# set-soft/ComfyUI-FLOAT_Optimized

Measured on AMD Instinct MI355X. Metric: 512x512 frames/sec end-to-end audio->video @50 ODE steps, higher is better.
Workload: dtype fp16; 1 GPU; configs[1]: 10 s audio + 512x512 portrait in HBM -> 250 frames in pinned host memory; appearance encoder + wav2vec2 audio encoder + FMT sampling (50 Euler evaluations/window, CFG a=2.0 e=1.0) + decode + D2H, through InferenceAgent.infer_device (the product call); nfe=51, frames_per_clip=250, fmt_dtype=fp16, dec_dtype=fp16, decode_batch=32, hip_graph=True, parallelism=replicas x1 (one clip per GPU), stage_overlap=off

## Files before the change

comfyui-float_optimized_amd/csrc/dec_kernels.hpp:

```cpp
#pragma once
#include "common.hpp"
#include <type_traits>

constexpr int kDecSatSites = 40;
typedef unsigned short dec_us2 __attribute__((ext_vector_type(2)));
typedef _Float16 dec_h2 __attribute__((ext_vector_type(2)));
template <class T>
__device__ __forceinline__ unsigned dec_cvt2(float a, float b, unsigned& m) {
  static_assert(T::is_fp16, "fp16 path");
  const unsigned u = __builtin_bit_cast(unsigned, dec_h2{(_Float16)a, (_Float16)b});
#ifndef DEC_NO_SAT
  m = __builtin_bit_cast(unsigned, __builtin_elementwise_max(__builtin_bit_cast(dec_us2, m), __builtin_bit_cast(dec_us2, u & 0x7fff7fffu)));
#endif
  return u;
}
template <class T>
__device__ __forceinline__ void dec_sat_flush(unsigned long long* ctr, unsigned& m) {
  if constexpr (T::is_fp16) {
    if ((m & 0xffffu) >= 0x7c00u || (m >> 16) >= 0x7c00u) atomicAdd(ctr, 1ull);
    m = 0u;
  }
}
template <class T>
__device__ __forceinline__ void dec_store4(typename T::elem* p, float a, float b, float c, float d, unsigned& m) {
// ... 1192 lines not shown
  issue(0);
  for (int chunk = 0; chunk < nchunks; ++chunk) {
    __syncthreads();
#pragma unroll
    for (int i = 0; i < NA; ++i) {
      const int e = tid + i * 256, p = e >> 2, ch = e & 3;
      if (p < NPIX) *reinterpret_cast<P8*>(sA + p * RB + (ch ^ ((p >> 1) & 3)) * CB) = ra[i];
    }
#pragma unroll
    for (int i = 0; i < NB; ++i) {
      const int e = tid + i * 256;
      if (e < NBC) {
        const int row = e >> 2, ch = e & 3;
        *reinterpret_cast<P8*>(sB + row * RB + (ch ^ ((row >> 1) & 3)) * CB) = rb[i];
      }
    }
    __syncthreads();
    if (chunk + 1 < nchunks) issue(chunk + 1);
    constexpr int kNum[4] = {1, 2, 2, 4};
    constexpr int kTap[4][4] = {{0, 0, 0, 0}, {1, 4, 0, 0}, {2, 6, 0, 0}, {3, 5, 7, 8}};
    constexpr int kCls[4][4] = {{0, 0, 0, 0}, {0, 1, 0, 0}, {0, 2, 0, 0}, {0, 1, 2, 3}};
#pragma unroll
    for (int sh = 0; sh < 4; ++sh) {
      P8 a[4];
#pragma unroll
      for (int mt = 0; mt < 4; ++mt)
        a[mt] = *reinterpret_cast<const P8*>(sA + ((sh & 1) ? (aaddr[mt][sh >> 1] >> 16) : (aaddr[mt][sh >> 1] & 0xffffu)));
#pragma unroll
      for (int u = 0; u < 4; ++u) {
        if (u < kNum[sh]) {
          const int t = kTap[sh][u], c = kCls[sh][u];
          P8 b[NT];
#pragma unroll
          for (int j = 0; j < NT; ++j) b[j] = *reinterpret_cast<const P8*>(sB + baddr + (t * BN + j * 16) * RB);
#pragma unroll
          for (int mt = 0; mt < 4; ++mt)
#pragma unroll
            for (int j = 0; j < NT; ++j) acc[c][mt][j] = T::mfma(b[j], a[mt], acc[c][mt][j]);
        }
      }
    }
  }
  float4 ed[NT];
  unsigned sm = 0u;
#pragma unroll
  for (int j = 0; j < NT; ++j) ed[j] = *reinterpret_cast<const float4*>(g.demod + (size_t)f * g.ldd + n0 + j * 16 + q * 4);
#pragma unroll
  for (int mt = 0; mt < 4; ++mt) {
    const int mpos = ty * 16 + w * 4 + mt, npos = tx * 16 + r16;
#pragma unroll
    for (int c = 0; c < 4; ++c) {
      const int u = 2 * mpos + (c >> 1), v = 2 * npos + (c & 1);
      if (u >= g.OH || v >= g.OW) continue;
      E* yp = reinterpret_cast<E*>(g.Y) + ((size_t)(f * g.OH + u) * g.OW + v) * g.Cout;
#pragma unroll
      for (int j = 0; j < NT; ++j) {
        const int co = n0 + j * 16 + q * 4;
        const float4 d = ed[j];
        dec_store4<T>(yp + co, acc[c][mt][j][0] * d.x, acc[c][mt][j][1] * d.y, acc[c][mt][j][2] * d.z, acc[c][mt][j][3] * d.w, sm);
      }
    }
  }
  dec_sat_flush<T>(g.sat, sm);
}

template <class T>
__global__ __launch_bounds__(256, T::is32 ? 1 : 2) void dec_zblur_kernel(ConvArgs g) {
  DEC_COPY_PROLOGUE(g, bid)
  DEC_PH_BEGIN
  typedef typename T::elem E;
  typedef typename T::pack8 P8;
  typedef float v2f __attribute__((ext_vector_type(2)));
  constexpr int EB = T::EB, RB = 32 * EB, CB = 8 * EB;
  constexpr int NT = 2, BN = 32, HW = 17, NPIX = HW * HW, NTAPS = 9;
  constexpr int NA = (NPIX * 4 + 255) / 256, NBROWS = NTAPS * BN, NB = (NBROWS * 4 + 255) / 256;
  extern __shared__ __attribute__((aligned(16))) unsigned char smem[];
  unsigned char* const sA = smem;
  unsigned char* const sB = smem + NPIX * RB;
  unsigned char* const sZ = smem;
  const int tid = threadIdx.x, lane = tid & 63, w = __builtin_amdgcn_readfirstlane(tid >> 6);
  const int r16 = lane & 15, q = lane >> 4;
  const int Wi = g.Wi, Cin = g.Cin;
  const int tiles_pf = g.tiles_x * g.tiles_y;
  unsigned grp = bid, cb = blockIdx.y;
  if (g.ncb) dec_group_cb(bid, g.ngroups, g.ncb, grp, cb);
  const int f = (int)grp / tiles_pf, rem = (int)grp - f * tiles_pf;
  const int ty = rem / g.tiles_x, tx = rem - ty * g.tiles_x;
  const int n0 = cb * BN;
  const int nchunks = Cin >> 5;
  const int iy0 = ty * 14 - 2, ix0 = tx * 14 - 2;

  const int ch = tid & 3;
  const bool interior = iy0 >= 0 && iy0 + HW <= g.Hi && ix0 >= 0 && ix0 + HW <= Wi;
  unsigned a_off[NA], a_lds[NA], a_bad = 0u;
#pragma unroll
  for (int i = 0; i < NA; ++i) {
    const int p = min((tid >> 2) + 64 * i, NPIX - 1);
    const int hy = p / HW, hx = p - hy * HW;
    const bool in = (unsigned)(iy0 + hy) < (unsigned)g.Hi && (unsigned)(ix0 + hx) < (unsigned)Wi;
    a_off[i] = (unsigned)((((in ? hy : 2) * Wi + (in ? hx : 2)) * Cin + ch * 8) * EB);
    a_lds[i] = (unsigned)(p * RB + (ch ^ ((hx >> 1) & 3)) * CB);
    a_bad |= (in ? 0u : 1u) << i;
  }
  const unsigned char* const Xo = reinterpret_cast<const unsigned char*>(g.X) + ((long long)(f * g.Hi + iy0) * Wi + ix0) * Cin * EB;
  const int brow = tid >> 2;
  const unsigned b_off = (unsigned)((((brow / BN) * g.Cout + brow % BN) * Cin + ch * 8) * EB);
  const int brow_l = min(brow + 64 * (NB - 1), NBROWS - 1);
  const unsigned b_off_l = (unsigned)((((brow_l / BN) * g.Cout + brow_l % BN) * Cin + ch * 8) * EB);
  const unsigned b_lds = (unsigned)(brow * RB + (ch ^ ((brow >> 1) & 3)) * CB);
  const unsigned b_lds_l = (unsigned)(brow_l * RB + (ch ^ ((brow_l >> 1) & 3)) * CB);
  const size_t b_round = (size_t)(64 / BN) * g.Cout * Cin * EB;
  const unsigned char* const Wn = reinterpret_cast<const unsigned char*>(g.Wt) + (size_t)n0 * Cin * EB;
  unsigned fa[2];
#pragma unroll
  for (int dx = 0; dx < 2; ++dx) fa[dx] = (unsigned)(((w * 4) * HW + r16 + dx) * RB + (q ^ (((r16 + dx) >> 1) & 3)) * CB);
  const unsigned fb = (unsigned)(r16 * RB + (q ^ ((r16 >> 1) & 3)) * CB);

  f32x4 acc[4][4][NT];
#pragma unroll
  for (int c = 0; c < 4; ++c)
#pragma unroll
    for (int i = 0; i < 4; ++i)
#pragma unroll
      for (int j = 0; j < NT; ++j) acc[c][i][j] = f32x4{0.f, 0.f, 0.f, 0.f};

  P8 ra[NA], rb[NB];
  float dm[NT];
  float4 b4, s4;
  auto issue = [&](int chunk) {
    const unsigned char* const Xc = Xo + (size_t)(chunk << 5) * EB;
#pragma unroll
    for (int i = 0; i < NA; ++i) ra[i] = *reinterpret_cast<const P8*>(Xc + a_off[i]);
    const unsigned char* const Wc = Wn + (size_t)(chunk << 5) * EB;
#pragma unroll
    for (int i = 0; i < NB - 1; ++i) rb[i] = *reinterpret_cast<const P8*>(Wc + i * b_round + b_off);
    rb[NB - 1] = *reinterpret_cast<const P8*>(Wc + b_off_l);
  };
  issue(0);
  DEC_PH(0);
  for (int chunk = 0; chunk < nchunks; ++chunk) {
    __syncthreads();
    if (interior) {
#pragma unroll
      for (int i = 0; i < NA; ++i) *reinterpret_cast<P8*>(sA + a_lds[i]) = ra[i];
    } else {
#pragma unroll
      for (int i = 0; i < NA; ++i) *reinterpret_cast<P8*>(sA + a_lds[i]) = ((a_bad >> i) & 1u) ? T::zero8() : ra[i];
    }
#pragma unroll
    for (int i = 0; i < NB - 1; ++i) *reinterpret_cast<P8*>(sB + b_lds + i * 64 * RB) = rb[i];
    *reinterpret_cast<P8*>(sB + b_lds_l) = rb[NB - 1];
    __syncthreads();
    DEC_PH(1);
    if (chunk + 1 < nchunks) {
      issue(chunk + 1);
    } else {
#pragma unroll
      for (int j = 0; j < NT; ++j) dm[j] = g.demod[(size_t)f * g.ldd + n0 + j * 16 + r16];
      const int co = n0 + (w & 1) * 16 + q * 4;
      b4 = *reinterpret_cast<const float4*>(g.bias + co);
      s4 = *reinterpret_cast<const float4*>(g.snext + (size_t)f * g.lds + co);
    }
    constexpr int kNum[4] = {1, 2, 2, 4};
    constexpr int kTap[4][4] = {{0, 0, 0, 0}, {1, 4, 0, 0}, {2, 6, 0, 0}, {3, 5, 7, 8}};
    constexpr int kCls[4][4] = {{0, 0, 0, 0}, {0, 1, 0, 0}, {0, 2, 0, 0}, {0, 1, 2, 3}};
#pragma unroll
    for (int sh = 0; sh < 4; ++sh) {
      P8 a[4];
#pragma unroll
      for (int mt = 0; mt < 4; ++mt) a[mt] = *reinterpret_cast<const P8*>(sA + fa[sh & 1] + (mt + (sh >> 1)) * HW * RB);
#pragma unroll
      for (int u = 0; u < 4; ++u) {
        if (u < kNum[sh]) {
          const int t = kTap[sh][u], c = kCls[sh][u];
          P8 b[NT];
#pragma unroll
          for (int j = 0; j < NT; ++j) b[j] = *reinterpret_cast<const P8*>(sB + fb + (t * BN + j * 16) * RB);
#pragma unroll
          for (int mt = 0; mt < 4; ++mt)
#pragma unroll
            for (int j = 0; j < NT; ++j) acc[c][mt][j] = T::mfma(a[mt], b[j], acc[c][mt][j]);
        }
      }
    }
    DEC_PH(2);
  }
  __syncthreads();
  unsigned sm = 0u;
  {
    const unsigned zw = (unsigned)(((8 * w) * 32 + r16) * RB + (q ^ ((r16 >> 1) & 3)) * CB);
#pragma unroll
    for (int mt = 0; mt < 4; ++mt)
#pragma unroll
      for (int pu = 0; pu < 2; ++pu)
#pragma unroll
        for (int j = 0; j < NT; ++j) {
          const f32x4 ev = acc[pu * 2][mt][j], od = acc[pu * 2 + 1][mt][j];
          const v2f d = v2f{dm[j], dm[j]};
          const v2f z0 = v2f{ev[0], od[0]} * d, z1 = v2f{ev[1], od[1]} * d, z2 = v2f{ev[2], od[2]} * d, z3 = v2f{ev[3], od[3]} * d;
          const float v[8] = {z0.x, z0.y, z1.x, z1.y, z2.x, z2.y, z3.x, z3.y};
          *reinterpret_cast<P8*>(sZ + zw + ((2 * mt + pu) * 32 + j * 16) * RB) = dec_pack8<T>(v, sm);
        }
  }
  __syncthreads();
  DEC_PH(3);
  {
    const int j2 = w & 1, half = w >> 1;
    const float f0 = g.fir[0], f1 = g.fir[1], f2 = g.fir[2], f3 = g.fir[3];
    asm volatile("" : "+v"(b4.x), "+v"(b4.y), "+v"(b4.z), "+v"(b4.w), "+v"(s4.x), "+v"(s4.y), "+v"(s4.z), "+v"(s4.w));
    const v2f bs[2] = {v2f{b4.x, b4.y}, v2f{b4.z, b4.w}};
    const v2f sn[2] = {v2f{s4.x * 1.4142135623730951f, s4.y * 1.4142135623730951f},
                       v2f{s4.z * 1.4142135623730951f, s4.w * 1.4142135623730951f}};
    const unsigned zrd = (unsigned)((((half * 14 + 1) * 32) + j2 * 16 + r16) * RB + (q ^ ((r16 >> 1) & 3)) * CB);
    unsigned char* const yt = reinterpret_cast<unsigned char*>(g.Y) + ((((size_t)f * g.OH + ty * 28) * g.OW + tx * 28) * g.Cout + n0) * EB;
    unsigned char* const sink = reinterpret_cast<unsigned char*>(g_dec_sink) + lane * 16;
    unsigned char* yp[2];
    unsigned ystep[2];
#pragma unroll
    for (int xt = 0; xt < 2; ++xt) {
#ifdef DEC_ZB_NOSTORE
      const bool ok = false;
#else
      const bool ok = 16 * xt + r16 < 28 && tx * 28 + 16 * xt + r16 < g.OW;
#endif
      yp[xt] = ok ? yt + (size_t)((16 * xt + r16) * g.Cout + j2 * 16 + q * 4) * EB : sink;
      ystep[xt] = ok ? (unsigned)(g.OW * g.Cout * EB) : 0u;
    }
    auto filter = [&](auto full_rows, auto symmetric) {
      constexpr bool FULL = decltype(full_rows)::value, SYM = decltype(symmetric)::value;
      P8 bx[2];
#pragma unroll
      for (int xt = 0; xt < 2; ++xt) {
        bx[xt] = T::zero8();
#pragma unroll
        for (int k = 0; k < 8; ++k) {
          const int t = 8 * q + k - (16 * xt + r16) - 1;
          float kv;
          if constexpr (SYM) kv = (t == 0 || t == 3) ? 0.25f : ((t == 1 || t == 2) ? 0.75f : 0.f);
          else kv = t == 0 ? f0 : (t == 1 ? f1 : (t == 2 ? f2 : (t == 3 ? f3 : 0.f)));
          T::set(bx[xt], k, (16 * xt + r16 < 28) ? kv : 0.f);
        }
      }
      P8 za[17];
#pragma unroll
      for (int r = 0; r < 17; ++r) za[r] = *reinterpret_cast<const P8*>(sZ + zrd + r * 32 * RB);
      f32x4 hd[17][2];
#pragma unroll
      for (int r = 0; r < 17; ++r)
#pragma unroll
        for (int xt = 0; xt < 2; ++xt) hd[r][xt] = T::mfma(za[r], bx[xt], f32x4{0.f, 0.f, 0.f, 0.f});
#pragma unroll
      for (int r = 3; r < 17; ++r) {
        const int yl = half * 14 + r - 3;
#pragma unroll
        for (int xt = 0; xt < 2; ++xt) {
          v2f v[2];
#pragma unroll
          for (int i = 0; i < 2; ++i) {
            const v2f h0 = v2f{hd[r - 3][xt][2 * i], hd[r - 3][xt][2 * i + 1]}, h1 = v2f{hd[r - 2][xt][2 * i], hd[r - 2][xt][2 * i + 1]};
            const v2f h2 = v2f{hd[r - 1][xt][2 * i], hd[r - 1][xt][2 * i + 1]}, h = v2f{hd[r][xt][2 * i], hd[r][xt][2 * i + 1]};
            v2f t;
            if constexpr (SYM) {
              t = 0.25f * (h0 + h) + bs[i];
              t = 0.75f * (h1 + h2) + t;
            } else {
              t = f0 * h0 + bs[i];
              t = f3 * h + t;
              t = f1 * h1 + t;
              t = f2 * h2 + t;
            }
            const v2f lo = 0.2f * t;
            v[i] = v2f{__builtin_amdgcn_fmed3f(t.x, lo.x, __builtin_inff()), __builtin_amdgcn_fmed3f(t.y, lo.y, __builtin_inff())} * sn[i];
          }
          unsigned char* const dst = (FULL || ty * 28 + yl < g.OH) ? yp[xt] + (unsigned)yl * ystep[xt] : sink;
          dec_store4<T>(reinterpret_cast<E*>(dst), v[0].x, v[0].y, v[1].x, v[1].y, sm);
        }
      }
      };
    const bool full = ty * 28 + 28 <= g.OH;
    if (g.fir_sym) {
      if (full) filter(std::true_type{}, std::true_type{});
      else filter(std::false_type{}, std::true_type{});
    } else {
      if (full) filter(std::true_type{}, std::false_type{});
      else filter(std::false_type{}, std::false_type{});
    }
  }
  dec_sat_flush<T>(g.sat, sm);
  DEC_PH(4);
  DEC_PH_COUNT(7);
  DEC_PH_END(0);
}

template <class T>
__global__ __launch_bounds__(256) void dec_blur_kernel(const typename T::elem* __restrict__ z, typename T::elem* __restrict__ out,
                                                       int F, int R, int C, const float* __restrict__ bias,
                                                       const float* __restrict__ snext, int lds, unsigned long long* sat,
                                                       float fir0, float fir1, float fir2, float fir3) {
  typedef typename T::pack8 P8;
  const int c8 = C >> 3, xq = R >> 2, yh = R >> 1;
  const size_t idx = (size_t)blockIdx.x * 256 + threadIdx.x;
  if (idx >= (size_t)F * yh * xq * c8) return;
  const int cg = (int)(idx % c8);
  size_t p = idx / c8;
  const int X0 = (int)(p % xq) * 4;
  p /= xq;
  const int Y0 = (int)(p % yh) * 2;
  const int f = (int)(p / yh);
  const int Z = R + 1;
  const float k1[4] = {fir0, fir1, fir2, fir3};
  float acc[2][4][8];
#pragma unroll
  for (int y = 0; y < 2; ++y)
#pragma unroll
    for (int j = 0; j < 4; ++j)
#pragma unroll
      for (int i = 0; i < 8; ++i) acc[y][j][i] = 0.f;
#pragma unroll
  for (int a = 0; a < 5; ++a) {
    const int zy = Y0 + a - 1;
    if (zy < 0 || zy > R) continue;
    P8 u[7];
#pragma unroll
    for (int b = 0; b < 7; ++b) {
      const int zx = X0 + b - 1;
      u[b] = (zx >= 0 && zx <= R) ? T::load8(z + ((size_t)(f * Z + zy) * Z + zx) * C + cg * 8) : T::zero8();
    }
    float h[4][8];
#pragma unroll
    for (int j = 0; j < 4; ++j)
#pragma unroll
      for (int i = 0; i < 8; ++i) h[j][i] = 0.f;
#pragma unroll
    for (int b = 0; b < 7; ++b) {
      float v[8];
#pragma unroll
      for (int i = 0; i < 8; ++i) v[i] = T::get(u[b], i);
#pragma unroll
      for (int j = 0; j < 4; ++j) {
        const int t = b - j;
        if (t >= 0 && t < 4) {
#pragma unroll
          for (int i = 0; i < 8; ++i) h[j][i] += k1[t] * v[i];
        }
      }
    }
#pragma unroll
    for (int y = 0; y < 2; ++y) {
      const int t = a - y;
      if (t >= 0 && t < 4) {
#pragma unroll
        for (int j = 0; j < 4; ++j)
#pragma unroll
          for (int i = 0; i < 8; ++i) acc[y][j][i] += k1[t] * h[j][i];
      }
    }
  }
  float bs[8], sn[8];
  unsigned sm = 0u;
#pragma unroll
  for (int i = 0; i < 8; ++i) {
    bs[i] = bias[cg * 8 + i];
    sn[i] = snext[(size_t)f * lds + cg * 8 + i];
  }
#pragma unroll
  for (int y = 0; y < 2; ++y)
#pragma unroll
    for (int j = 0; j < 4; ++j) {
      float ov[8];
#pragma unroll
      for (int i = 0; i < 8; ++i) ov[i] = fh_lrelu_s2(acc[y][j][i] + bs[i]) * sn[i];
      T::store8(out + ((size_t)(f * R + Y0 + y) * R + X0 + j) * C + cg * 8, dec_pack8<T>(ov, sm));
    }
// ... 289 lines not shown
```

comfyui-float_optimized_amd/csrc/dec_launch.hpp:

```cpp
#pragma once
#include "dec_pack.hpp"
#include "tuning.hpp"

namespace {

enum DecOut : int { kOutNone = 0, kOutHWC = 1, kOutRawCHW = 2, kOutU8 = 3, kOutI420 = 4 };
inline size_t out_frame_bytes(DecOut mode, int size) {
  const size_t npix = (size_t)size * size;
  return mode == kOutI420 ? npix + npix / 2 : npix * 3 * (mode == kOutU8 ? sizeof(uint8_t) : sizeof(float));
}

enum RideKind : int { kRideUpconv = 0, kRideConv2 = 1, kRideFlow = 2, kRideKinds = 3 };

struct RideCopy {
  const char* src = nullptr;
  char* dst = nullptr;
  char* dst_host = nullptr;
  size_t left16 = 0;
  double wleft = 0.0;

  static double weight(const DecTune& tn, int R, int kind) {
    if (tn.ride_equal) return 1.0;
    const int li = R == 64 ? 0 : R == 128 ? 1 : R == 256 ? 2 : R == 512 ? 3 : -1;
    return li < 0 ? 250.0 : tn.ride_w[li][kind];
// ... 128 lines not shown
    c.sy = c.sx = 2;
    c.py = pu, c.px = pv;
    c.ntaps = t.n, c.tap0 = first[2 * pu + pv];
    for (int i = 0; i < t.n; ++i) c.dy[i] = t.dy[i], c.dx[i] = t.dx[i];
    return c;
  }
};

inline ConvArgs conv_args_of(const Styled& s, const void* X, void* Y, int F, int Hi, int Wi, int OH, int OW, Rows demod, unsigned long long* sat) {
  ConvArgs g;
  memset(&g, 0, sizeof(g));
  g.X = X, g.Y = Y;
  g.Wt = s.W;
  g.demod = demod.p, g.ldd = demod.ld;
  g.sat = sat, g.F = F;
  g.Hi = Hi, g.Wi = Wi;
  g.Cin = s.cin, g.Cout = s.cout;
  g.OH = OH, g.OW = OW;
  return g;
}

template <class T>
int launch_conv(const DecLaunch& cx, const ConvGeom& c, const Styled& s, const void* X, void* Y, int F, Rows demod, Rows snext,
                unsigned long long* sat, const void* wfrag = nullptr, float* oflow = nullptr) {
  typedef typename T::elem E;
  constexpr size_t RB = 32 * T::EB;
  const DecTune& tn = cx.tn;
  ConvArgs g = conv_args_of(s, X, Y, F, c.Hi, c.Wi, c.OH, c.OW, demod, sat);
  g.Wt = reinterpret_cast<const E*>(s.W) + (size_t)c.tap0 * s.cout * s.cin;
  g.wfrag = wfrag, g.oflow = oflow;
  g.bias = c.act ? s.abias : nullptr, g.act = c.act ? 1 : 0;
  g.snext = snext.p, g.lds = snext.ld;
  g.Ho = c.Ho, g.Wo = c.Wo;
  g.sy = c.sy, g.sx = c.sx, g.py = c.py, g.px = c.px;
  g.ntaps = c.ntaps;
  for (int t = 0; t < c.ntaps; ++t) g.dy[t] = (signed char)c.dy[t], g.dx[t] = (signed char)c.dx[t];
  const int dymin = *std::min_element(c.dy, c.dy + c.ntaps), dymax = *std::max_element(c.dy, c.dy + c.ntaps);
  const int dxmin = *std::min_element(c.dx, c.dx + c.ntaps), dxmax = *std::max_element(c.dx, c.dx + c.ntaps);
  const int tdim = conv_tile(c.Ho, c.Wo);
  g.lth = g.ltw = ilog2(tdim);
  g.lnf = 8 - 2 * g.lth;
  g.dymin = dymin, g.dxmin = dxmin;
  g.hh = tdim + dymax - dymin, g.hw = tdim + dxmax - dxmin;
  g.tiles_x = (c.Wo + tdim - 1) / tdim, g.tiles_y = (c.Ho + tdim - 1) / tdim;
  const int nf = 1 << g.lnf;
  const int fblocks = (F + nf - 1) / nf;
  const int npix = nf * g.hh * g.hw;
  FH_REQUIRE(npix * 4 <= 9 * 256, "conv halo tile too large (%d pixels)", npix);
  const int bn = conv_bn(tn, s, tdim);
  FH_REQUIRE(s.cout % bn == 0 && s.cin % 32 == 0, "conv channels (%d -> %d) not tileable", s.cin, s.cout);
  const int ty_taps = dymax - dymin + 1, tx_taps = dxmax - dxmin + 1;
  void (*kern)(ConvArgs) = nullptr;
  dim3 grid;
  size_t smem;
  if (tdim == 16 && ty_taps == 3 && tx_taps == 3 && c.ntaps == 9 && c.Ho % 16 == 0 && c.Wo % 16 == 0 && c.Ho == c.Hi && c.Wo == c.Wi) {
    const int total = g.tiles_x * g.tiles_y * F;
    g.tpw = tn.tpw ? tn.tpw : (total >= 16384 ? 4 : (total >= 4096 ? 2 : 1));
    smem = (size_t)(15 + ty_taps) * (15 + tx_taps) * RB + (size_t)c.ntaps * bn * RB + 3 * bn * sizeof(float);
    g.ct = cx.take(c.Ho, kRideConv2);
    grid = dim3((total + g.tpw - 1) / g.tpw + g.ct.nwg, s.cout / bn);
    if (tn.cb_order && s.cout / bn > 1) {
      g.ngroups = (unsigned)((total + g.tpw - 1) / g.tpw);
      g.ncb = (unsigned)(s.cout / bn);
      grid = dim3(g.ngroups * g.ncb + g.ct.nwg, 1);
    }
    const bool db = !oflow && !T::is32 && ((bn == 64 && (tn.conv_db & 1)) || (bn == 32 && (tn.conv_db & 2)));
    FH_REQUIRE(!oflow || s.cout == bn, "ToFlow epilogue needs the layer's %d output channels in one block of %d", s.cout, bn);
    for_each_conv16<T>([&](auto k, int kbn, bool kdb, bool kflow) {
      if (kbn == bn && kdb == db && kflow == (oflow != nullptr)) kern = k;
    });
    smem = db ? 2 * smem : cx.smem(smem);
  } else {
    FH_REQUIRE(!oflow, "ToFlow epilogue: only on the 16x16-tile 3x3 kernel (%d x %d)", c.Ho, c.Wo);
    smem = (size_t)npix * RB + (size_t)c.ntaps * bn * RB;
    grid = dim3(g.tiles_x * g.tiles_y * fblocks, s.cout / bn);
    kern = bn == 64 ? dec_conv_kernel<T, 4> : dec_conv_kernel<T, 2>;
  }
  FH_REQUIRE(kern, "no 3x3 conv kernel with %d channels per workgroup", bn);
  fh_launch_prof(1, kern, grid, dim3(256), smem, cx.st, g);
  FH_CHECK_HIP(hipGetLastError());
  return FLOAT_OK;
}

template <class T>
int launch_upconv(const DecLaunch& cx, const Styled& up, int Ri, int n, const void* x_in, void* Zb, void* U, void** U_out, Rows demod,
                  Rows snext, unsigned long long* sat) {
  typedef typename T::elem E;
  constexpr size_t RB = 32 * T::EB;
  const DecTune& tn = cx.tn;
  const int R = 2 * Ri;
  int rc;
  if (R >= tn.zblur_min && up.cout % 32 == 0 && up.cin % 32 == 0) {
    ConvArgs z = conv_args_of(up, x_in, Zb, n, Ri, Ri, R, R, demod, sat);
    z.bias = up.abias;
    z.snext = snext.p, z.lds = snext.ld;
    for (int b = 0; b < 4; ++b) z.fir[b] = up.fir[b];
    z.fir_sym = (up.fir[0] == 0.25f && up.fir[1] == 0.75f && up.fir[2] == 0.75f && up.fir[3] == 0.25f) ? 1 : 0;
    z.tiles_x = z.tiles_y = (R + 27) / 28;
    z.ct = cx.take(R, kRideUpconv);
    dim3 grid(z.tiles_x * z.tiles_y * n + z.ct.nwg, up.cout / 32);
    if (tn.cb_order && up.cout / 32 > 1) {
      z.ngroups = (unsigned)(z.tiles_x * z.tiles_y * n);
      z.ncb = (unsigned)(up.cout / 32);
      grid = dim3(z.ngroups * z.ncb + z.ct.nwg, 1);
    }
    fh_launch_prof(1, dec_zblur_kernel<T>, grid, dim3(256), cx.smem(32 * 32 * RB), cx.st, z);
    *U_out = Zb;
    FH_CHECK_HIP(hipGetLastError());
    return FLOAT_OK;
  }
  if (Ri + 1 > 8 && up.cout % 32 == 0 && !tn.no_zfuse) {
    ConvArgs z = conv_args_of(up, x_in, Zb, n, Ri, Ri, R + 1, R + 1, demod, sat);
    z.tiles_x = z.tiles_y = (Ri + 1 + 15) / 16;
    dim3 grid(z.tiles_x * z.tiles_y * n, up.cout / 32);
    fh_launch_prof(1, dec_zconv4_kernel<T>, grid, dim3(256), 17 * 17 * RB + 9 * 32 * RB, cx.st, z);
  } else {
    const DecLaunch plain{tn, nullptr, cx.st};
    for (int pu = 0; pu < 2; ++pu)
      for (int pv = 0; pv < 2; ++pv)
        if ((rc = launch_conv<T>(plain, ConvGeom::up_class(Ri, pu, pv), up, x_in, Zb, n, demod, Rows{}, sat))) return rc;
  }
  const size_t tot = (size_t)n * (R / 2) * (R / 4) * (up.cout / 8);
  hipLaunchKernelGGL((dec_blur_kernel<T>), dim3((unsigned)((tot + 255) / 256)), dim3(256), 0, cx.st, reinterpret_cast<const E*>(Zb),
                     reinterpret_cast<E*>(U), n, R, up.cout, up.abias, snext.p, snext.ld, sat, up.fir[0], up.fir[1], up.fir[2], up.fir[3]);
  *U_out = U;
  FH_CHECK_HIP(hipGetLastError());
  return FLOAT_OK;
}

inline FlowArgs flow_args_of(const Level& L, const float* styles, int ld_s, int F) {
  FlowArgs g;
  memset(&g, 0, sizeof(g));
  g.feat = L.feat;
  memcpy(g.upk_flow, L.upk_flow, sizeof(g.upk_flow));
  memcpy(g.upk_rgb, L.upk_rgb, sizeof(g.upk_rgb));
  g.wflow = L.wflow, g.bflow = L.bflow;
  g.sflow = styles + L.style_off, g.ld_s = ld_s;
  g.wrgb = L.wrgb, g.grgb = L.grgb;
  g.b1 = L.b1, g.b2 = L.b2, g.lin = L.lin;
  g.F = F, g.R = L.R, g.C = L.C;
  return g;
}

inline bool flowlast_takes_i420(int R) { return R >= 128 && R % 128 == 0; }

inline int launch_rgb8_to_i420(const DecLaunch& cx, const unsigned char* rgb, void* out, int n, int R) {
  FH_REQUIRE(R % 8 == 0, "I420 frames: %d px is not a multiple of 8", R);
  const size_t lanes = (size_t)n * (R / 2) * (R / 8);
  hipLaunchKernelGGL(dec_rgb8_to_i420_kernel, dim3((unsigned)((lanes + 255) / 256)), dim3(256), 0, cx.st, rgb,
                     static_cast<unsigned char*>(out), n, R);
  FH_CHECK_HIP(hipGetLastError());
  return FLOAT_OK;
}

template <class T>
int launch_flow(const DecLaunch& cx, FlowArgs g) {
  const DecTune& tn = cx.tn;
  if (g.oflow) {
    const int runs = (g.R * g.R + 255) / 256;
    g.ct = cx.take(g.R, kRideFlow);
    FH_REQUIRE(g.final_mode != kOutU8 || (g.R * g.R) % 256 == 0, "8-bit frames: %d x %d pixels are not whole runs of 256", g.R, g.R);
    FH_REQUIRE(g.final_mode != kOutI420 || flowlast_takes_i420(g.R), "I420 frames: %d px is not whole blocks of 128 columns", g.R);
    void (*kern)(FlowArgs);
    switch (g.final_mode) {
      case kOutU8: kern = dec_flowlast_kernel<T, true>; break;
      case kOutI420: kern = dec_flowlast_kernel<T, false, true>; break;
      default: kern = dec_flowlast_kernel<T>;
    }
    hipLaunchKernelGGL(kern, dim3(runs * g.F + g.ct.nwg), dim3(256), (size_t)tn.lds_pad, cx.st, g);
    FH_CHECK_HIP(hipGetLastError());
    return FLOAT_OK;
  }
  const int R = g.R, n = g.F;
  const int lpp = g.C / 8, gpb = 256 / lpp;
  const int pix = (tn.flow_pix == 1 || tn.flow_pix == 2 || tn.flow_pix == 4) ? tn.flow_pix : (lpp <= 8 ? 4 : 2);
  const int step = gpb * pix;
  const int max_bx = (R * R + step - 1) / step;
  int bx = std::max(1, std::min(max_bx, (tn.flow_wgs + n - 1) / n));
  if (bx >= 8) bx &= ~7;
  g.band_pix = ((R * R + bx - 1) / bx + step - 1) / step * step;
  g.nbands = bx = (R * R + g.band_pix - 1) / g.band_pix;
  g.ct = cx.take(R, kRideFlow);
  const size_t pad = tn.lds_pad > 14 * 1024 ? (size_t)tn.lds_pad - 14 * 1024 : 0;
  const dim3 grid(bx * n + g.ct.nwg);
  for_each_flow<T>([&](auto kern, int kpix, bool klast) {
// ... 46 lines not shown
```

comfyui-float_optimized_amd/csrc/tuning.hpp:

```cpp
#pragma once
#include <stdio.h>
#include <stdlib.h>
#include <string.h>

#include <algorithm>
#include <string>

inline int env_int(const char* name, int dflt, int lo, int hi) {
  const char* v = getenv(name);
  if (!v || !*v) return dflt;
  char* end = nullptr;
  const long x = strtol(v, &end, 10);
  return (end && *end == 0 && x >= lo && x <= hi) ? (int)x : dflt;
}
inline int env_atoi(const char* name, int dflt) {
  const char* v = getenv(name);
  return v ? atoi(v) : dflt;
}
inline bool env_set(const char* name) { return getenv(name) != nullptr; }
inline int env_scan(const char* s, int* v) { int n = 0; return sscanf(s, "%d%n", v, &n) == 1 ? n : 0; }
inline int env_scan(const char* s, double* v) { int n = 0; return sscanf(s, "%lf%n", v, &n) == 1 ? n : 0; }
template <class V>
int env_list(const char* name, V* v, int n, char sep = ',') {
  const char* s = getenv(name);
// ... 11 lines not shown
struct LayerPlan {
  int v[3] = {0, 0, 0};
  bool on() const { return v[0] > 0; }
};

enum { RB_QKV = 0, RB_PROJ, RB_FC1, RB_FC2 };

struct FmtTune {
  bool wide = true;
  int wide_variant = 7;
  bool big = true;
  bool rb = true;
  int rb_touch = 16;
  struct Rb {
    int n = 0, shape = -1, ksplit = 1;
  } rb_layer[4];
  int full_nw = 8;
  int plan[6] = {0, 0, 0, 0, 0, 0};
  LayerPlan plan_layer[4];
  int fc2_split = 4;
  int proj_split = 0;
  int touch = 230;
  bool hoist = true;
  int zgroup = 0;
  int ln_rows = 1;
  int attn_qpw = 8, attn_lpq = 16;
  bool no_tokblk = false;
  int attnproj = 0;
  int mega = 0;
  int mega_stamp_wg = 0;
  bool pack_host = false;

  static FmtTune from_env() {
    FmtTune t;
    t.wide = env_atoi("FLOAT_FMT_WIDE", 1) != 0;
    t.wide_variant = env_atoi("FLOAT_FMT_WIDE_VARIANT", t.wide_variant);
    t.big = env_atoi("FLOAT_FMT_BIG", 1) != 0;
    t.rb = env_atoi("FLOAT_FMT_RB", 1) != 0;
    t.rb_touch = env_atoi("FLOAT_FMT_RB_TOUCH", t.rb_touch);
    static const char* const layers[4] = {"QKV", "PROJ", "FC1", "FC2"};
    for (int l = 0; l < 4; ++l) {
      const std::string s = layers[l];
      int rb[2] = {-1, 1};
      t.rb_layer[l].n = env_list(("FLOAT_FMT_RB_" + s).c_str(), rb, 2);
      t.rb_layer[l].shape = rb[0];
      t.rb_layer[l].ksplit = rb[1];
      env_list(("FLOAT_FMT_PLAN_" + s).c_str(), t.plan_layer[l].v, 3);
    }
    t.full_nw = env_atoi("FLOAT_FMT_FULL_NW", t.full_nw);
    env_list("FLOAT_FMT_PLAN", t.plan, 6);
    t.fc2_split = env_atoi("FLOAT_FMT_FC2_SPLIT", t.fc2_split);
    t.proj_split = env_atoi("FLOAT_FMT_PROJ_SPLIT", t.proj_split);
    t.touch = env_atoi("FLOAT_FMT_TOUCH", t.touch);
    t.hoist = env_atoi("FLOAT_FMT_HOIST", 1) != 0;
    t.zgroup = std::max(0, env_atoi("FLOAT_FMT_ZGROUP", 0));
    t.ln_rows = std::max(1, std::min(4, env_atoi("FLOAT_FMT_LN_ROWS", 1)));
    int attn[2] = {t.attn_qpw, t.attn_lpq};
    env_list("FLOAT_FMT_ATTN", attn, 2);
    t.attn_lpq = attn[1] == 16 ? 16 : 8;
    t.attn_qpw = std::max(1, std::min(512 / t.attn_lpq, attn[0]));
    t.no_tokblk = env_set("FLOAT_FMT_NO_TOKBLK");
    t.attnproj = env_atoi("FLOAT_FMT_ATTNPROJ", 0);
    t.mega = env_atoi("FLOAT_FMT_MEGA", 0);
    t.mega_stamp_wg = env_atoi("FLOAT_FMT_MEGA_STAMP_WG", 0);
    t.pack_host = env_atoi("FLOAT_PACK_HOST", 0) != 0;
    return t;
  }
};

struct DecTune {
  int lds_pad = 0;
  unsigned ride_wgs = 16;
  int ride_min_res = 64;
  unsigned ride_pace = 3;
  bool ride_equal = false;
  double ride_w[4][3] = {{170, 140, 50}, {170, 155, 100}, {220, 200, 180}, {300, 250, 120}};
  int ride_tail = 0;
#ifdef DEC_STAMPS
  int ride_test = 0;
#endif
  bool cb_order = true;
  int conv_bn = 64, conv_bn_lo = 32;
  int tpw = 0;
  int conv_db = 0;
  bool no_zfuse = false;
  int zblur_min = 64;
  int flow_pix = 0;
  int flow_wgs = 2048;
  bool flow_epi = true;
  bool yuv_fused = true;
  bool write_pyr = false;
  bool copy_memcpy = false;
  bool short_first = true;
  bool style_norm = true;

  static DecTune from_env() {
    DecTune t;
    t.lds_pad = env_int("FLOAT_DEC_LDS_PAD", 0, 0, 160 * 1024);
    t.ride_wgs = (unsigned)env_int("FLOAT_DEC_RIDE_WGS", 16, 0, 64) / 8 * 8;
    t.ride_min_res = env_int("FLOAT_DEC_RIDE_MIN_RES", 64, 64, 512);
    t.ride_pace = (unsigned)env_int("FLOAT_DEC_RIDE_PACE", 3, 0, 64);
    t.ride_equal = env_set("FLOAT_DEC_RIDE_EQUAL");
    double w[12];
    if (env_list("FLOAT_DEC_RIDE_W", w, 12, ' ') == 12)
      for (int i = 0; i < 12; ++i)
        if (w[i] > 0.0 && w[i] < 1e6) t.ride_w[i / 3][i % 3] = w[i];
    t.ride_tail = env_atoi("FLOAT_DEC_RIDE_TAIL", 0);
#ifdef DEC_STAMPS
    t.ride_test = env_int("FLOAT_DEC_RIDE_TEST", 0, 0, 2);
#endif
    t.cb_order = env_atoi("FLOAT_DEC_CB_ORDER", 1) != 0;
    t.conv_bn = env_int("FLOAT_DEC_CONV_BN", 64, 32, 64);
    t.conv_bn_lo = env_int("FLOAT_DEC_CONV_BN_LO", 32, 32, 64);
    t.tpw = env_int("FLOAT_DEC_TPW", 0, 0, 4096);
    t.conv_db = env_int("FLOAT_DEC_CONV_DB", 0, 0, 3);
    t.no_zfuse = env_set("FLOAT_DEC_NO_ZFUSE");
    t.zblur_min = env_int("FLOAT_DEC_ZBLUR_MIN", 64, 16, 4096);
    t.flow_pix = env_int("FLOAT_DEC_FLOW_PIX", 0, 0, 4);
    t.flow_wgs = env_int("FLOAT_DEC_FLOW_WGS", 2048, 8, 1 << 20);
    t.flow_epi = env_int("FLOAT_DEC_FLOW_EPI", 1, 0, 1) != 0;
    t.yuv_fused = env_int("FLOAT_DEC_YUV_FUSED", 1, 0, 1) != 0;
    t.write_pyr = env_set("FLOAT_DEC_WRITE_PYR");
    const char* copy = getenv("FLOAT_DEC_COPY");
    t.copy_memcpy = copy && !strcmp(copy, "memcpy");
    t.short_first = env_int("FLOAT_DEC_SHORT_FIRST", 1, 0, 1) != 0;
    t.style_norm = env_int("FLOAT_DEC_STYLE_NORM", 1, 0, 1) != 0;
    return t;
  }
};

struct EncTune {
  bool no_tiles = false;
  static EncTune from_env() { return EncTune{env_set("FLOAT_ENC_NO_TILES")}; }
};

struct AudTune {
  bool attn_mfma = true;
  static AudTune from_env() { return AudTune{env_atoi("FLOAT_AUD_ATTN_MFMA", 1) != 0}; }
};
```

Measured before the change: 2348 frames/s.

## Make zblur upconv kernel persistent over multiple tiles with cross-tile prefetch

```diff
diff --git a/comfyui-float_optimized_amd/csrc/dec_kernels.hpp b/comfyui-float_optimized_amd/csrc/dec_kernels.hpp
--- a/comfyui-float_optimized_amd/csrc/dec_kernels.hpp
+++ b/comfyui-float_optimized_amd/csrc/dec_kernels.hpp
@@ -1298,33 +1298,31 @@
   const int r16 = lane & 15, q = lane >> 4;
   const int Wi = g.Wi, Cin = g.Cin;
   const int tiles_pf = g.tiles_x * g.tiles_y;
+  const int total = tiles_pf * g.F;
+  const int nchunks = Cin >> 5;
   unsigned grp = bid, cb = blockIdx.y;
   if (g.ncb) dec_group_cb(bid, g.ngroups, g.ncb, grp, cb);
-  const int f = (int)grp / tiles_pf, rem = (int)grp - f * tiles_pf;
-  const int ty = rem / g.tiles_x, tx = rem - ty * g.tiles_x;
+  const int tile0 = (int)grp * g.tpw;
+  const int ntile = min(g.tpw, total - tile0);
   const int n0 = cb * BN;
-  const int nchunks = Cin >> 5;
-  const int iy0 = ty * 14 - 2, ix0 = tx * 14 - 2;
+  if (ntile <= 0) return;
 
   const int ch = tid & 3;
-  const bool interior = iy0 >= 0 && iy0 + HW <= g.Hi && ix0 >= 0 && ix0 + HW <= Wi;
-  unsigned a_off[NA], a_lds[NA], a_bad = 0u;
+  const int yhi = g.Hi - (14 * (g.tiles_y - 1) - 2), xhi = Wi - (14 * (g.tiles_x - 1) - 2);
+  unsigned a_off[NA], a_lds[NA], a_edge = 0u;
 #pragma unroll
   for (int i = 0; i < NA; ++i) {
     const int p = min((tid >> 2) + 64 * i, NPIX - 1);
     const int hy = p / HW, hx = p - hy * HW;
-    const bool in = (unsigned)(iy0 + hy) < (unsigned)g.Hi && (unsigned)(ix0 + hx) < (unsigned)Wi;
-    a_off[i] = (unsigned)((((in ? hy : 2) * Wi + (in ? hx : 2)) * Cin + ch * 8) * EB);
+    a_off[i] = (unsigned)(((hy * Wi + hx) * Cin + ch * 8) * EB);
     a_lds[i] = (unsigned)(p * RB + (ch ^ ((hx >> 1) & 3)) * CB);
-    a_bad |= (in ? 0u : 1u) << i;
-  }
-  const unsigned char* const Xo = reinterpret_cast<const unsigned char*>(g.X) + ((long long)(f * g.Hi + iy0) * Wi + ix0) * Cin * EB;
+    const unsigned m = (hy < 2 ? 1u : 0u) | (hy >= yhi ? 2u : 0u) | (hx < 2 ? 4u : 0u) | (hx >= xhi ? 8u : 0u);
+    a_edge |= m << (4 * i);
+  }
   const int brow = tid >> 2;
   const unsigned b_off = (unsigned)((((brow / BN) * g.Cout + brow % BN) * Cin + ch * 8) * EB);
-  const int brow_l = min(brow + 64 * (NB - 1), NBROWS - 1);
-  const unsigned b_off_l = (unsigned)((((brow_l / BN) * g.Cout + brow_l % BN) * Cin + ch * 8) * EB);
   const unsigned b_lds = (unsigned)(brow * RB + (ch ^ ((brow >> 1) & 3)) * CB);
-  const unsigned b_lds_l = (unsigned)(brow_l * RB + (ch ^ ((brow_l >> 1) & 3)) * CB);
+  static_assert(NBROWS - 64 * (NB - 1) == 32, "the last staging round of the weight slab is 32 rows = two waves");
   const size_t b_round = (size_t)(64 / BN) * g.Cout * Cin * EB;
   const unsigned char* const Wn = reinterpret_cast<const unsigned char*>(g.Wt) + (size_t)n0 * Cin * EB;
   unsigned fa[2];
@@ -1332,79 +1330,127 @@
   for (int dx = 0; dx < 2; ++dx) fa[dx] = (unsigned)(((w * 4) * HW + r16 + dx) * RB + (q ^ (((r16 + dx) >> 1) & 3)) * CB);
   const unsigned fb = (unsigned)(r16 * RB + (q ^ ((r16 >> 1) & 3)) * CB);
 
+  const int j2 = w & 1, half = w >> 1;
+  const float f0 = g.fir[0], f1 = g.fir[1], f2 = g.fir[2], f3 = g.fir[3];
+  const unsigned st_row = (unsigned)(g.OW * g.Cout * EB);
+
+  int sf, sty, stx, schunk = 0;
+  {
+    sf = tile0 / tiles_pf;
+    const int rem = tile0 - sf * tiles_pf;
+    sty = rem / g.tiles_x;
+    stx = rem - sty * g.tiles_x;
+  }
+  int cf = sf, cty = sty, ctx = stx;
+  unsigned s_edge = 0u;
+
+  P8 ra[NA], rb[NB];
+  auto issue = [&]() {
+    const unsigned edge = (sty == 0 ? 1u : 0u) | (sty == g.tiles_y - 1 ? 2u : 0u) | (stx == 0 ? 4u : 0u) | (stx == g.tiles_x - 1 ? 8u : 0u);
+    s_edge = edge;
+    const long long org = ((long long)(sf * g.Hi + sty * 14 - 2) * Wi + stx * 14 - 2) * Cin + (schunk << 5);
+    const unsigned char* const Xo = reinterpret_cast<const unsigned char*>(g.X) + org * EB;
+    unsigned off[NA];
+#pragma unroll
+    for (int i = 0; i < NA; ++i) off[i] = a_off[i];
+    if (edge != 0u) {
+      const unsigned hit = a_edge & (edge * 0x11111111u);
+      int t = tid;
+      asm volatile("" : "+v"(t));
+      const unsigned a_safe = (unsigned)(((2 * Wi + 2) * Cin + (t & 3) * 8) * EB);
+#pragma unroll
+      for (int i = 0; i < NA; ++i) off[i] = ((hit >> (4 * i)) & 15u) ? a_safe : off[i];
+    }
+#pragma unroll
+    for (int i = 0; i < NA; ++i) ra[i] = *reinterpret_cast<const P8*>(Xo + off[i]);
+    const unsigned char* const Wc = Wn + (size_t)(schunk << 5) * EB;
+#pragma unroll
+    for (int i = 0; i < NB - 1; ++i) rb[i] = *reinterpret_cast<const P8*>(Wc + i * b_round + b_off);
+    if (w < 2) rb[NB - 1] = *reinterpret_cast<const P8*>(Wc + (NB - 1) * b_round + b_off);
+    if (++schunk == nchunks) {
+      schunk = 0;
+      if (++stx == g.tiles_x) {
+        stx = 0;
+        if (++sty == g.tiles_y) {
+          sty = 0;
+          ++sf;
+        }
+      }
+    }
+  };
+
   f32x4 acc[4][4][NT];
-#pragma unroll
-  for (int c = 0; c < 4; ++c)
-#pragma unroll
-    for (int i = 0; i < 4; ++i)
-#pragma unroll
-      for (int j = 0; j < NT; ++j) acc[c][i][j] = f32x4{0.f, 0.f, 0.f, 0.f};
-
-  P8 ra[NA], rb[NB];
   float dm[NT];
   float4 b4, s4;
-  auto issue = [&](int chunk) {
-    const unsigned char* const Xc = Xo + (size_t)(chunk << 5) * EB;
-#pragma unroll
-    for (int i = 0; i < NA; ++i) ra[i] = *reinterpret_cast<const P8*>(Xc + a_off[i]);
-    const unsigned char* const Wc = Wn + (size_t)(chunk << 5) * EB;
-#pragma unroll
-    for (int i = 0; i < NB - 1; ++i) rb[i] = *reinterpret_cast<const P8*>(Wc + i * b_round + b_off);
-    rb[NB - 1] = *reinterpret_cast<const P8*>(Wc + b_off_l);
-  };
-  issue(0);
+  issue();
   DEC_PH(0);
-  for (int chunk = 0; chunk < nchunks; ++chunk) {
+  for (int tile = 0; tile < ntile; ++tile) {
+#pragma unroll
+    for (int c = 0; c < 4; ++c)
+#pragma unroll
+      for (int i = 0; i < 4; ++i)
+#pragma unroll
+        for (int j = 0; j < NT; ++j) acc[c][i][j] = f32x4{0.f, 0.f, 0.f, 0.f};
+    for (int chunk = 0; chunk < nchunks; ++chunk) {
+      __syncthreads();
+      if (s_edge == 0u) {
+#pragma unroll
+        for (int i = 0; i < NA; ++i) *reinterpret_cast<P8*>(sA + a_lds[i]) = ra[i];
+      } else {
+        const unsigned hit = a_edge & (s_edge * 0x11111111u);
+#pragma unroll
+        for (int i = 0; i < NA; ++i) *reinterpret_cast<P8*>(sA + a_lds[i]) = ((hit >> (4 * i)) & 15u) ? T::zero8() : ra[i];
+      }
+#pragma unroll
+      for (int i = 0; i < NB - 1; ++i) *reinterpret_cast<P8*>(sB + b_lds + i * 64 * RB) = rb[i];
+      if (w < 2) *reinterpret_cast<P8*>(sB + b_lds + (NB - 1) * 64 * RB) = rb[NB - 1];
+      __syncthreads();
+      DEC_PH(1);
+      if (chunk + 1 == nchunks) {
+        int el = lane;
+        asm volatile("" : "+v"(el));
+        const unsigned char* const dmb = reinterpret_cast<const unsigned char*>(g.demod + (size_t)cf * g.ldd + n0);
+#pragma unroll
+        for (int j = 0; j < NT; ++j) dm[j] = *reinterpret_cast<const float*>(dmb + (unsigned)((j * 16 + (el & 15)) * 4));
+        if (tile + 1 < ntile) issue();
+      } else {
+        issue();
+      }
+      constexpr int kNum[4] = {1, 2, 2, 4};
+      constexpr int kTap[4][4] = {{0, 0, 0, 0}, {1, 4, 0, 0}, {2, 6, 0, 0}, {3, 5, 7, 8}};
+      constexpr int kCls[4][4] = {{0, 0, 0, 0}, {0, 1, 0, 0}, {0, 2, 0, 0}, {0, 1, 2, 3}};
+#pragma unroll
+      for (int sh = 0; sh < 4; ++sh) {
+        P8 a[4];
+#pragma unroll
+        for (int mt = 0; mt < 4; ++mt) a[mt] = *reinterpret_cast<const P8*>(sA + fa[sh & 1] + (mt + (sh >> 1)) * HW * RB);
+#pragma unroll
+        for (int u = 0; u < 4; ++u) {
+          if (u < kNum[sh]) {
+            const int t = kTap[sh][u], c = kCls[sh][u];
+            P8 b[NT];
+#pragma unroll
+            for (int j = 0; j < NT; ++j) b[j] = *reinterpret_cast<const P8*>(sB + fb + (t * BN + j * 16) * RB);
+#pragma unroll
+            for (int mt = 0; mt < 4; ++mt)
+#pragma unroll
+              for (int j = 0; j < NT; ++j) acc[c][mt][j] = T::mfma(a[mt], b[j], acc[c][mt][j]);
+          }
+        }
+      }
+      DEC_PH(2);
+    }
     __syncthreads();
-    if (interior) {
-#pragma unroll
-      for (int i = 0; i < NA; ++i) *reinterpret_cast<P8*>(sA + a_lds[i]) = ra[i];
-    } else {
-#pragma unroll
-      for (int i = 0; i < NA; ++i) *reinterpret_cast<P8*>(sA + a_lds[i]) = ((a_bad >> i) & 1u) ? T::zero8() : ra[i];
-    }
-#pragma unroll
-    for (int i = 0; i < NB - 1; ++i) *reinterpret_cast<P8*>(sB + b_lds + i * 64 * RB) = rb[i];
-    *reinterpret_cast<P8*>(sB + b_lds_l) = rb[NB - 1];
-    __syncthreads();
-    DEC_PH(1);
-    if (chunk + 1 < nchunks) {
-      issue(chunk + 1);
-    } else {
-#pragma unroll
-      for (int j = 0; j < NT; ++j) dm[j] = g.demod[(size_t)f * g.ldd + n0 + j * 16 + r16];
-      const int co = n0 + (w & 1) * 16 + q * 4;
-      b4 = *reinterpret_cast<const float4*>(g.bias + co);
-      s4 = *reinterpret_cast<const float4*>(g.snext + (size_t)f * g.lds + co);
-    }
-    constexpr int kNum[4] = {1, 2, 2, 4};
-    constexpr int kTap[4][4] = {{0, 0, 0, 0}, {1, 4, 0, 0}, {2, 6, 0, 0}, {3, 5, 7, 8}};
-    constexpr int kCls[4][4] = {{0, 0, 0, 0}, {0, 1, 0, 0}, {0, 2, 0, 0}, {0, 1, 2, 3}};
-#pragma unroll
-    for (int sh = 0; sh < 4; ++sh) {
-      P8 a[4];
-#pragma unroll
-      for (int mt = 0; mt < 4; ++mt) a[mt] = *reinterpret_cast<const P8*>(sA + fa[sh & 1] + (mt + (sh >> 1)) * HW * RB);
-#pragma unroll
-      for (int u = 0; u < 4; ++u) {
-        if (u < kNum[sh]) {
-          const int t = kTap[sh][u], c = kCls[sh][u];
-          P8 b[NT];
-#pragma unroll
-          for (int j = 0; j < NT; ++j) b[j] = *reinterpret_cast<const P8*>(sB + fb + (t * BN + j * 16) * RB);
-#pragma unroll
-          for (int mt = 0; mt < 4; ++mt)
-#pragma unroll
-            for (int j = 0; j < NT; ++j) acc[c][mt][j] = T::mfma(a[mt], b[j], acc[c][mt][j]);
-        }
-      }
-    }
-    DEC_PH(2);
-  }
-  __syncthreads();
-  unsigned sm = 0u;
-  {
-    const unsigned zw = (unsigned)(((8 * w) * 32 + r16) * RB + (q ^ ((r16 >> 1) & 3)) * CB);
+    unsigned sm = 0u;
+    int zl = lane;
+    asm volatile("" : "+v"(zl));
+    const int zr16 = zl & 15, zq = zl >> 4;
+    const unsigned zw = (unsigned)(((8 * w) * 32 + zr16) * RB + (zq ^ ((zr16 >> 1) & 3)) * CB);
+    {
+      const int co = n0 + j2 * 16;
+      b4 = *reinterpret_cast<const float4*>(reinterpret_cast<const unsigned char*>(g.bias + co) + (unsigned)(zq * 16));
+      s4 = *reinterpret_cast<const float4*>(reinterpret_cast<const unsigned char*>(g.snext + (size_t)cf * g.lds + co) + (unsigned)(zq * 16));
+    }
 #pragma unroll
     for (int mt = 0; mt < 4; ++mt)
 #pragma unroll
@@ -1417,94 +1463,109 @@
           const float v[8] = {z0.x, z0.y, z1.x, z1.y, z2.x, z2.y, z3.x, z3.y};
           *reinterpret_cast<P8*>(sZ + zw + ((2 * mt + pu) * 32 + j * 16) * RB) = dec_pack8<T>(v, sm);
         }
-  }
-  __syncthreads();
-  DEC_PH(3);
-  {
-    const int j2 = w & 1, half = w >> 1;
-    const float f0 = g.fir[0], f1 = g.fir[1], f2 = g.fir[2], f3 = g.fir[3];
-    asm volatile("" : "+v"(b4.x), "+v"(b4.y), "+v"(b4.z), "+v"(b4.w), "+v"(s4.x), "+v"(s4.y), "+v"(s4.z), "+v"(s4.w));
-    const v2f bs[2] = {v2f{b4.x, b4.y}, v2f{b4.z, b4.w}};
-    const v2f sn[2] = {v2f{s4.x * 1.4142135623730951f, s4.y * 1.4142135623730951f},
-                       v2f{s4.z * 1.4142135623730951f, s4.w * 1.4142135623730951f}};
-    const unsigned zrd = (unsigned)((((half * 14 + 1) * 32) + j2 * 16 + r16) * RB + (q ^ ((r16 >> 1) & 3)) * CB);
-    unsigned char* const yt = reinterpret_cast<unsigned char*>(g.Y) + ((((size_t)f * g.OH + ty * 28) * g.OW + tx * 28) * g.Cout + n0) * EB;
-    unsigned char* const sink = reinterpret_cast<unsigned char*>(g_dec_sink) + lane * 16;
-    unsigned char* yp[2];
-    unsigned ystep[2];
-#pragma unroll
-    for (int xt = 0; xt < 2; ++xt) {
-#ifdef DEC_ZB_NOSTORE
-      const bool ok = false;
-#else
-      const bool ok = 16 * xt + r16 < 28 && tx * 28 + 16 * xt + r16 < g.OW;
-#endif
-      yp[xt] = ok ? yt + (size_t)((16 * xt + r16) * g.Cout + j2 * 16 + q * 4) * EB : sink;
-      ystep[xt] = ok ? (unsigned)(g.OW * g.Cout * EB) : 0u;
-    }
-    auto filter = [&](auto full_rows, auto symmetric) {
-      constexpr bool FULL = decltype(full_rows)::value, SYM = decltype(symmetric)::value;
+    __syncthreads();
+    DEC_PH(3);
+    {
+      asm volatile("" : "+v"(b4.x), "+v"(b4.y), "+v"(b4.z), "+v"(b4.w), "+v"(s4.x), "+v"(s4.y), "+v"(s4.z), "+v"(s4.w));
+      const v2f bs[2] = {v2f{b4.x, b4.y}, v2f{b4.z, b4.w}};
+      const v2f sn[2] = {v2f{s4.x * 1.4142135623730951f, s4.y * 1.4142135623730951f},
+                         v2f{s4.z * 1.4142135623730951f, s4.w * 1.4142135623730951f}};
+      const unsigned zrd = (unsigned)((((half * 14 + 1) * 32) + j2 * 16 + zr16) * RB + (zq ^ ((zr16 >> 1) & 3)) * CB);
       P8 bx[2];
 #pragma unroll
       for (int xt = 0; xt < 2; ++xt) {
         bx[xt] = T::zero8();
+        const bool in = 16 * xt + zr16 < 28;
+        const unsigned u0 = in ? __float_as_uint(f0) : 0u, u1 = in ? __float_as_uint(f1) : 0u;
+        const unsigned u2 = in ? __float_as_uint(f2) : 0u, u3 = in ? __float_as_uint(f3) : 0u;
 #pragma unroll
         for (int k = 0; k < 8; ++k) {
-          const int t = 8 * q + k - (16 * xt + r16) - 1;
-          float kv;
-          if constexpr (SYM) kv = (t == 0 || t == 3) ? 0.25f : ((t == 1 || t == 2) ? 0.75f : 0.f);
-          else kv = t == 0 ? f0 : (t == 1 ? f1 : (t == 2 ? f2 : (t == 3 ? f3 : 0.f)));
-          T::set(bx[xt], k, (16 * xt + r16 < 28) ? kv : 0.f);
-        }
-      }
-      P8 za[17];
-#pragma unroll
-      for (int r = 0; r < 17; ++r) za[r] = *reinterpret_cast<const P8*>(sZ + zrd + r * 32 * RB);
-      f32x4 hd[17][2];
-#pragma unroll
-      for (int r = 0; r < 17; ++r)
-#pragma unroll
-        for (int xt = 0; xt < 2; ++xt) hd[r][xt] = T::mfma(za[r], bx[xt], f32x4{0.f, 0.f, 0.f, 0.f});
-#pragma unroll
-      for (int r = 3; r < 17; ++r) {
-        const int yl = half * 14 + r - 3;
-#pragma unroll
-        for (int xt = 0; xt < 2; ++xt) {
-          v2f v[2];
-#pragma unroll
-          for (int i = 0; i < 2; ++i) {
-            const v2f h0 = v2f{hd[r - 3][xt][2 * i], hd[r - 3][xt][2 * i + 1]}, h1 = v2f{hd[r - 2][xt][2 * i], hd[r - 2][xt][2 * i + 1]};
-            const v2f h2 = v2f{hd[r - 1][xt][2 * i], hd[r - 1][xt][2 * i + 1]}, h = v2f{hd[r][xt][2 * i], hd[r][xt][2 * i + 1]};
-            v2f t;
-            if constexpr (SYM) {
-              t = 0.25f * (h0 + h) + bs[i];
-              t = 0.75f * (h1 + h2) + t;
-            } else {
-              t = f0 * h0 + bs[i];
-              t = f3 * h + t;
-              t = f1 * h1 + t;
-              t = f2 * h2 + t;
+          const int t = 8 * zq + k - (16 * xt + zr16) - 1;
+          const unsigned kb = (t == 0 ? u0 : 0u) | (t == 1 ? u1 : 0u) | (t == 2 ? u2 : 0u) | (t == 3 ? u3 : 0u);
+          T::set(bx[xt], k, __uint_as_float(kb));
+        }
+      }
+      unsigned char* const yt = reinterpret_cast<unsigned char*>(g.Y) + ((((size_t)cf * g.OH + cty * 28) * g.OW + ctx * 28) * g.Cout + n0) * EB;
+      unsigned char* const sink = reinterpret_cast<unsigned char*>(g_dec_sink) + zl * 16;
+      unsigned char* yp[2];
+      unsigned ystep[2];
+#pragma unroll
+      for (int xt = 0; xt < 2; ++xt) {
+#ifdef DEC_ZB_NOSTORE
+        const bool ok = false;
+#else
+        const bool ok = 16 * xt + zr16 < 28 && ctx * 28 + 16 * xt + zr16 < g.OW;
+#endif
+        yp[xt] = ok ? yt + (unsigned)(((16 * xt + zr16) * g.Cout + j2 * 16 + zq * 4) * EB) : sink;
+        ystep[xt] = ok ? st_row : 0u;
+      }
+      auto filter = [&](auto full_rows, auto symmetric) {
+        constexpr bool FULL = decltype(full_rows)::value, SYM = decltype(symmetric)::value;
+        constexpr int kStage[5] = {0, 5, 9, 13, 17};
+        P8 za[17];
+        f32x4 hd[17][2];
+#pragma unroll
+        for (int r = kStage[0]; r < kStage[1]; ++r) za[r] = *reinterpret_cast<const P8*>(sZ + zrd + r * 32 * RB);
+#pragma unroll
+        for (int st = 0; st < 4; ++st) {
+#pragma unroll
+          for (int r = kStage[st]; r < kStage[st + 1]; ++r)
+#pragma unroll
+            for (int xt = 0; xt < 2; ++xt) hd[r][xt] = T::mfma(za[r], bx[xt], f32x4{0.f, 0.f, 0.f, 0.f});
+          if (st < 3) {
+#pragma unroll
+            for (int r = kStage[st + 1]; r < kStage[st + 2]; ++r) za[r] = *reinterpret_cast<const P8*>(sZ + zrd + r * 32 * RB);
+          }
+#pragma unroll
+          for (int r = (kStage[st] < 3 ? 3 : kStage[st]); r < kStage[st + 1]; ++r) {
+            const int yl = half * 14 + r - 3;
+#pragma unroll
+            for (int xt = 0; xt < 2; ++xt) {
+              v2f v[2];
+#pragma unroll
+              for (int i = 0; i < 2; ++i) {
+                const v2f h0 = v2f{hd[r - 3][xt][2 * i], hd[r - 3][xt][2 * i + 1]}, h1 = v2f{hd[r - 2][xt][2 * i], hd[r - 2][xt][2 * i + 1]};
+                const v2f h2 = v2f{hd[r - 1][xt][2 * i], hd[r - 1][xt][2 * i + 1]}, h = v2f{hd[r][xt][2 * i], hd[r][xt][2 * i + 1]};
+                v2f t;
+                if constexpr (SYM) {
+                  t = 0.25f * (h0 + h) + bs[i];
+                  t = 0.75f * (h1 + h2) + t;
+                } else {
+                  t = f0 * h0 + bs[i];
+                  t = f3 * h + t;
+                  t = f1 * h1 + t;
+                  t = f2 * h2 + t;
+                }
+                const v2f lo = 0.2f * t;
+                v[i] = v2f{__builtin_amdgcn_fmed3f(t.x, lo.x, __builtin_inff()), __builtin_amdgcn_fmed3f(t.y, lo.y, __builtin_inff())} * sn[i];
+              }
+              unsigned char* const dst = (FULL || cty * 28 + yl < g.OH) ? yp[xt] + (unsigned)yl * ystep[xt] : sink;
+              dec_store4<T>(reinterpret_cast<E*>(dst), v[0].x, v[0].y, v[1].x, v[1].y, sm);
             }
-            const v2f lo = 0.2f * t;
-            v[i] = v2f{__builtin_amdgcn_fmed3f(t.x, lo.x, __builtin_inff()), __builtin_amdgcn_fmed3f(t.y, lo.y, __builtin_inff())} * sn[i];
           }
-          unsigned char* const dst = (FULL || ty * 28 + yl < g.OH) ? yp[xt] + (unsigned)yl * ystep[xt] : sink;
-          dec_store4<T>(reinterpret_cast<E*>(dst), v[0].x, v[0].y, v[1].x, v[1].y, sm);
-        }
-      }
+          __builtin_amdgcn_sched_barrier(0);
+        }
       };
-    const bool full = ty * 28 + 28 <= g.OH;
-    if (g.fir_sym) {
-      if (full) filter(std::true_type{}, std::true_type{});
-      else filter(std::false_type{}, std::true_type{});
-    } else {
-      if (full) filter(std::true_type{}, std::false_type{});
-      else filter(std::false_type{}, std::false_type{});
-    }
-  }
-  dec_sat_flush<T>(g.sat, sm);
-  DEC_PH(4);
-  DEC_PH_COUNT(7);
+      const bool full = cty * 28 + 28 <= g.OH;
+      if (g.fir_sym) {
+        if (full) filter(std::true_type{}, std::true_type{});
+        else filter(std::false_type{}, std::true_type{});
+      } else {
+        if (full) filter(std::true_type{}, std::false_type{});
+        else filter(std::false_type{}, std::false_type{});
+      }
+    }
+    dec_sat_flush<T>(g.sat, sm);
+    if (++ctx == g.tiles_x) {
+      ctx = 0;
+      if (++cty == g.tiles_y) {
+        cty = 0;
+        ++cf;
+      }
+    }
+    DEC_PH(4);
+    DEC_PH_COUNT(7);
+  }
   DEC_PH_END(0);
 }
 
diff --git a/comfyui-float_optimized_amd/csrc/dec_launch.hpp b/comfyui-float_optimized_amd/csrc/dec_launch.hpp
--- a/comfyui-float_optimized_amd/csrc/dec_launch.hpp
+++ b/comfyui-float_optimized_amd/csrc/dec_launch.hpp
@@ -234,6 +234,8 @@
   return FLOAT_OK;
 }
 
+inline int zb_tpw_of(int ) { return 1; }
+
 template <class T>
 int launch_upconv(const DecLaunch& cx, const Styled& up, int Ri, int n, const void* x_in, void* Zb, void* U, void** U_out, Rows demod,
                   Rows snext, unsigned long long* sat) {
@@ -249,10 +251,13 @@
     for (int b = 0; b < 4; ++b) z.fir[b] = up.fir[b];
     z.fir_sym = (up.fir[0] == 0.25f && up.fir[1] == 0.75f && up.fir[2] == 0.75f && up.fir[3] == 0.25f) ? 1 : 0;
     z.tiles_x = z.tiles_y = (R + 27) / 28;
+    const int total = z.tiles_x * z.tiles_y * n;
+    z.tpw = tn.zb_tpw ? tn.zb_tpw : zb_tpw_of(total);
+    const int groups = (total + z.tpw - 1) / z.tpw;
     z.ct = cx.take(R, kRideUpconv);
-    dim3 grid(z.tiles_x * z.tiles_y * n + z.ct.nwg, up.cout / 32);
+    dim3 grid(groups + z.ct.nwg, up.cout / 32);
     if (tn.cb_order && up.cout / 32 > 1) {
-      z.ngroups = (unsigned)(z.tiles_x * z.tiles_y * n);
+      z.ngroups = (unsigned)groups;
       z.ncb = (unsigned)(up.cout / 32);
       grid = dim3(z.ngroups * z.ncb + z.ct.nwg, 1);
     }
diff --git a/comfyui-float_optimized_amd/csrc/tuning.hpp b/comfyui-float_optimized_amd/csrc/tuning.hpp
--- a/comfyui-float_optimized_amd/csrc/tuning.hpp
+++ b/comfyui-float_optimized_amd/csrc/tuning.hpp
@@ -117,6 +117,7 @@
   bool cb_order = true;
   int conv_bn = 64, conv_bn_lo = 32;
   int tpw = 0;
+  int zb_tpw = 0;
   int conv_db = 0;
   bool no_zfuse = false;
   int zblur_min = 64;
@@ -148,6 +149,7 @@
     t.conv_bn = env_int("FLOAT_DEC_CONV_BN", 64, 32, 64);
     t.conv_bn_lo = env_int("FLOAT_DEC_CONV_BN_LO", 32, 32, 64);
     t.tpw = env_int("FLOAT_DEC_TPW", 0, 0, 4096);
+    t.zb_tpw = env_int("FLOAT_DEC_ZB_TPW", 0, 0, 4096);
     t.conv_db = env_int("FLOAT_DEC_CONV_DB", 0, 0, 3);
     t.no_zfuse = env_set("FLOAT_DEC_NO_ZFUSE");
     t.zblur_min = env_int("FLOAT_DEC_ZBLUR_MIN", 64, 16, 4096);
```

Result: no change. 2342 frames/s (-0.3%).
